# broadinstitute/colab-repeat-finder

Hardware: AMD Instinct MI355X
Metric: Gbp/s scanned (motif 1-50) (higher is better)
Workload: dtype u32 bit planes (2-bit bases)

## Files before the change

colab-repeat-finder_amd/csrc/scan_vertical.hip:

```cpp
#include <algorithm>
#include <cstdio>
#include <cstdlib>
#include <utility>
#include <vector>

#include "prf_host.h"
#include "prf_static_for.h"
#include "scan_vertical.h"
#include "verify_impl.h"

namespace {

#include "vscan_common.h"
#include "vscan_verify.h"
#include "vscan_tasks.h"

__device__ __forceinline__ void set_prio(u32 p) {
#ifdef PRF_NO_PRIO
    return;
#endif
    if (p == 0u) __builtin_amdgcn_s_setprio(0);
    else if (p == 1u) __builtin_amdgcn_s_setprio(1);
    else if (p == 2u) __builtin_amdgcn_s_setprio(2);
    else __builtin_amdgcn_s_setprio(3);
}

__device__ __forceinline__ u32 lds_add(prf_lds_u32 *p, u32 v) {
    return __hip_atomic_fetch_add(p, v, __ATOMIC_RELAXED, __HIP_MEMORY_SCOPE_WORKGROUP);
}

__device__ __forceinline__ void dma16(const void *src_lane, u32 lds_byte_off) {
    __builtin_amdgcn_global_load_lds((prf_glb_cvoid *)src_lane, (prf_lds_void *)(prf_smem + lds_byte_off), 16, 0, 0);
}

template <int NC>
struct NextRegs {
    static constexpr int extra = NC - 64;
    static constexpr u32 n_extra = (u32)(2 * RG * extra);
    static_assert(n_extra <= (u32)NTH, "one virtual-lane slot per thread");
    static_assert((RG * extra) % 64 == 0, "virtual-lane staging: one plane per wave");
    prf_u32x4 ev, en;
    u32 entry;

    __device__ __forceinline__ static prf_u32x4 ld16(const void *ubase, u32 byte_off) {
        return *reinterpret_cast<const prf_u32x4 *>(reinterpret_cast<const char *>(ubase) + byte_off);
    }
    __device__ __forceinline__ void load(const prf_vscan_args &g, u32 e, int tid, int wave, u32 r1_off) {
        e = (u32)__builtin_amdgcn_readfirstlane((int)e);
        entry = e;
        const u64 tile = e & ~PRF_LAUNCH_MIXED;
        const prf_u32x4 *ph = reinterpret_cast<const prf_u32x4 *>(g.VH) + tile * (RG * 64), *pL = reinterpret_cast<const prf_u32x4 *>(g.VL) + tile * (RG * 64);
        u32 ut = (u32)tid;
        asm volatile("" : "+v"(ut));
        {
            const u32 p = (u32)wave >> 1, rg0 = ((u32)wave & 1u) * 4u;
            const prf_u32x4 *pp = p ? pL : ph;
            const u32 l16 = (ut & 63u) * 16u;
            static_for<0, 4>([&](auto ic) {
                constexpr u32 i = (u32)decltype(ic)::value;
                dma16(reinterpret_cast<const char *>(pp) + ((rg0 + i) * 64u * 16u + l16), r1_off + ((p * RG + rg0 + i) * (u32)NC) * 16u);
            });
        }
        const prf_u32x4 z = {0, 0, 0, 0};
        ev = z;
        en = z;
        if (ut < n_extra) {
            const u32 pw = (u32)__builtin_amdgcn_readfirstlane((int)(ut / (u32)(RG * extra)));
            const u32 erg = (ut / (u32)extra) % (u32)RG, el = ut % (u32)extra;
            const u32 i0 = (erg * 64u + el) * 16u, i1 = i0 + (u32)(RG * 64) * 16u;
            if (pw == 0) {
                ev = ld16(ph, i0);
                en = ld16(ph, i1);
            } else {
                ev = ld16(pL, i0);
                en = ld16(pL, i1);
            }
        }
    }
    __device__ __forceinline__ void clear() {
        const prf_u32x4 z = {0, 0, 0, 0};
        ev = en = z;
        entry = 0;
    }
    __device__ __forceinline__ void store(prf_lds_u4 *vimg, int tid) const {
        const u32 sx = (u32)tid;
        if (sx < n_extra) {
            const u32 p = sx / (u32)(RG * extra), erg = (sx / (u32)extra) % (u32)RG, el = sx % (u32)extra;
            vimg[p * RG * NC + erg * (u32)NC + 64u + el] = (ev >> 1) | (en << 31);
        }
    }
};

__device__ __forceinline__ u32 vscan_skip(const prf_vscan_args &g) {
#ifdef PRF_DIAG
    return g.skip;
#else
    (void)g;
    return 0u;
#endif
}

template <int NC>
__global__ __launch_bounds__(NTH, 6) void prf_vscan_kernel(prf_vscan_args g) {
    constexpr u32 R1_OFF = (u32)SMEM_HDR, R1_BYTES = (u32)(2 * RG * NC * 16);
    constexpr u32 RECS_OFF = R1_OFF + R1_BYTES, KEYS_OFF = RECS_OFF + (u32)REC_CAP * 8u, SLOW_OFF = KEYS_OFF + 2u * (u32)ROW_CAP_LDS * 4u,
                  HOTW_OFF = SLOW_OFF + (u32)SLOW_CAP * 16u, BITEMS_OFF = HOTW_OFF + (u32)FLAG_CAP * 2u;
    static_assert(SLOW_CAP * 16 >= 256, "the all-N stream masks lie in the deferred candidates' list");
    static_assert(2 * LW * 8 <= (int)R1_BYTES, "the window of the linear planes must fit the image's region");
    static_assert((2 * LW / 2 + 63) / 64 <= 5 * MAX_WAVES, "window pieces per wave");
    prf_lds_u4 *vimg = (prf_lds_u4 *)(prf_smem + R1_OFF);
    prf_lds_u64 *recs = (prf_lds_u64 *)(prf_smem + RECS_OFF);
    prf_lds_u32 *keys = (prf_lds_u32 *)(prf_smem + KEYS_OFF);
    prf_lds_u32 *nostart = (prf_lds_u32 *)(prf_smem + SLOW_OFF);
    prf_lds_u32 *hotw = (prf_lds_u32 *)(prf_smem + HOTW_OFF);
    prf_lds_u32 *bitems = (prf_lds_u32 *)(prf_smem + BITEMS_OFF);

    const int tid0 = (int)threadIdx.x;
    const int wave = __builtin_amdgcn_readfirstlane(tid0 >> 6);
    auto entry_of = [&](u32 sl) -> u32 { return g.flat_base != ~0u ? g.flat_base + sl : g.launch_list[sl]; };

    set_prio(g.plan.prio & 3u);
    NextRegs<NC> sr;
    sr.load(g, entry_of(blockIdx.x), tid0, wave, R1_OFF);
    for (u32 v = (u32)tid0; v < 8u * g.plan.n_tasks; v += (u32)NTH) {
        const prf_vtask task = g.plan.tasks[v >> 3];
        const u32 kk = v & 7u;
        if (task.kind == 0 && ((task.valid >> kk) & 1u))
            bitems[(u32)task.item0 + (u32)__builtin_popcount((u32)task.valid & ((1u << kk) - 1u))] = ((u32)task.k0 + kk) | ((u32)task.stride << 16);
    }
    {
        prf_lds_u32 *cof_lds = bitems + g.plan.n_group_k;
        for (int i = tid0; i < (int)g.plan.cof_words; i += NTH) cof_lds[i] = prf_cof_table.v[i];
    }
    if (tid0 == 0) {
        TileCtx *tcw = reinterpret_cast<TileCtx *>(prf_smem);
        tcw->H = g.H; tcw->L = g.L; tcw->X = g.X;
        tcw->E = g.E;
        tcw->slab_cap = g.slab_cap;
        tcw->min_repeats = g.min_repeats;
        tcw->min_span = g.min_span;
        tcw->lin_off = R1_OFF;
        tcw->keys_off = KEYS_OFF;
        tcw->slow_off = SLOW_OFF;
        tcw->k_exact0 = g.plan.k_exact0;
        tcw->cof_off = BITEMS_OFF + 4u * g.plan.n_group_k;
    }

    const u32 xcd = blockIdx.x & 7u;
    const u32 first_ticket = (gridDim.x - xcd + 7u) >> 3;
    u64 *ticket_word = g.counters + (PRF_CNT_SHARD0 + xcd * PRF_CNT_SHARD_STRIDE + PRF_SH_TILE_TICKET);
    prf_lds_u32 *next_words = (prf_lds_u32 *)(prf_smem + HDR_NEXT);
    u32 slot_next = 0;
    u32 parity = 0;
    prf_lds_u32 *wg_stats = (prf_lds_u32 *)(prf_smem + HDR_STATS);
    if (tid0 == 0) wg_stats[0] = wg_stats[1] = 0;
    for (u32 slot = blockIdx.x; slot < g.n_launch; slot = slot_next, parity ^= 1u) {
    int wave_s = wave;
    asm volatile("" : "+s"(wave_s));
    u32 ones = ~0u;
    asm volatile("" : "+s"(ones));
    int tid = wave_s * 64 + (int)__builtin_amdgcn_mbcnt_hi(ones, __builtin_amdgcn_mbcnt_lo(ones, 0u));
    asm volatile("" : "+v"(tid));
    const int lane = tid & 63;
    const u32 entry = sr.entry;
    const bool hasx = (entry & PRF_LAUNCH_MIXED) != 0;
    const u64 tile = entry & ~PRF_LAUNCH_MIXED;
    prf_lds_u32 *cnt = smem_cnt(parity);

    PRF_STAMP(0);
#ifdef PRF_STAMPS
    if (g.dbg && lane == 0) g.dbg[((u64)slot * MAX_WAVES + wave) * 16 + 12] = __builtin_amdgcn_s_memrealtime();
#endif
    set_prio(g.plan.prio & 3u);
    {
        sr.store(vimg, tid);
        if (hasx && tid < 64) {
            const u32 *px = reinterpret_cast<const u32 *>(g.X + tile * PRF_TILE_WORDS);
            u32 m = 0;
#pragma unroll 1
            for (u32 b0 = 0; b0 < 32u; b0 += 8u) {
                u32 v[8];
                static_for<0, 8>([&](auto bc) { v[decltype(bc)::value] = *(prf_glb_cu32 *)(px + ((b0 + (u32)decltype(bc)::value) * 64u + (u32)tid)); });
                static_for<0, 8>([&](auto bc) { m |= (v[decltype(bc)::value] == ~0u ? 1u : 0u) << (b0 + (u32)decltype(bc)::value); });
            }
            nostart[tid] = m;
        }
        if (tid < 8) cnt[tid] = 0;
        if (tid == 0) {
            TileCtx *tcw = reinterpret_cast<TileCtx *>(prf_smem);
            tcw->w0 = tile * PRF_TILE_WORDS - LIN_PRE;
            tcw->xz_lo = hasx ? 0 : tile * PRF_TILE;
            tcw->xz_hi = hasx ? 0 : (tile + 2) * PRF_TILE;
            tcw->slab = (prf_glb_u64 *)(g.slabs + (u64)slot * g.slab_cap);
            tcw->tile_base = tile * PRF_TILE;
            tcw->has_lin = 0u;
            tcw->cnt_off = (u32)HDR_CNT + 32u * parity;
        }
    }
    PRF_STAMP(1);
    __syncthreads();
    PRF_STAMP(2);

    set_prio(((g.plan.slack_waves >> wave) & 1u) ? (g.plan.prio >> 4) & 3u : (g.plan.prio >> 2) & 3u);
    Emit em;
    em.recs = recs;
    em.cnt = cnt;
    em.lane = lane;
#ifdef PRF_STAMPS
    u64 *task_dbg = g.dbg ? g.dbg + ((u64)slot * MAX_WAVES + wave) * 16 : nullptr;
#else
    u64 *task_dbg = nullptr;
#endif
    {
        u32 allow = hasx ? ~nostart[lane] : ~0u;
        if (vscan_skip(g) & 1u) allow = 0u;
        run_tasks<NC>((prf_lds_cu4 *)vimg, hotw, g.plan, wave, lane, hasx, allow, em, task_dbg);
    }
    constexpr u32 WIN_UNITS = (u32)LW;
    constexpr u32 WIN_PIECES = (WIN_UNITS + 63u) / 64u;
    static_assert(WIN_PIECES == 17, "the window's pieces are dealt 9 + 8 to the first two waves to arrive");
    prf_u32x4 wv[9];
    u32 order = 0;
    {
        if (lane == 0) order = atomicAdd((u32 *)(cnt + CNT_ROWS0), 1u);
        order = (u32)__builtin_amdgcn_readfirstlane((int)order);
        const long long w0 = (long long)(tile * PRF_TILE_WORDS) - LIN_PRE;
        const u64 *wh = g.H + w0, *wl = g.L + w0;
        const prf_u32x4 z = {0, 0, 0, 0};
        static_for<0, 9>([&](auto ic) { wv[decltype(ic)::value] = z; });
        if (order < 2u) {
            const u32 first = order * 9u, n = order ? 8u : 9u;
            static_for<0, 9>([&](auto ic) {
                constexpr u32 i = (u32)decltype(ic)::value;
                if (i < n) {
                    const u32 u = (first + i) * 64u + (u32)lane;
                    const u64 *src = u < (u32)LW / 2u ? wh + 2u * u : wl + 2u * (u - (u32)LW / 2u);
                    if (u < WIN_UNITS) wv[i] = *reinterpret_cast<const prf_u32x4 *>(src);
                }
            });
        }
    }
    u64 ticket = 0;
    const bool ticket_thread = order == 0u && lane == 0;
    if (ticket_thread) ticket = atomicAdd(ticket_word, 1ull);
    PRF_STAMP(3);
    __syncthreads();
    {
        if (order < 2u) {
            const u32 first = order * 9u, n = order ? 8u : 9u;
            static_for<0, 9>([&](auto ic) {
                constexpr u32 i = (u32)decltype(ic)::value;
                if (i < n) {
                    const u32 u = (first + i) * 64u + (u32)lane;
                    if (u < WIN_UNITS) *(prf_lds_u4 *)(prf_smem + R1_OFF + 16u * u) = wv[i];
                }
            });
        }
        const u32 n0 = cnt[CNT_ROWS];
        for (u32 i = (u32)tid; i < (u32)ROW_CAP_LDS; i += (u32)NTH)
            if (i >= n0) keys[i] = 0xFFFFFFFFu;
        if (tid == 0) {
            reinterpret_cast<TileCtx *>(prf_smem)->has_lin = 1u;
            cnt[CNT_ROWS0] = n0;
            cnt[CNT_LONG0] = cnt[CNT_LONG];
        }
    }
    u32 slot_pre = 0, entry_pre = entry;
    if (ticket_thread) {
        slot_pre = (first_ticket + (u32)ticket) * 8u + xcd;
        if (slot_pre < g.n_launch) entry_pre = entry_of(slot_pre);
    }
    __syncthreads();
    PRF_STAMP(4);

    set_prio(wave < MAX_WAVES / 2 ? (g.plan.prio >> 6) & 3u : (g.plan.prio >> 8) & 3u);
    const u32 *xw = hasx ? reinterpret_cast<const u32 *>(g.X + ((long long)(tile * PRF_TILE_WORDS) - LIN_PRE)) : nullptr;
    typedef const unsigned short __attribute__((address_space(3))) prf_lds_cu16;
    u32 n_recs = cnt[CNT_RECS], n_flags = cnt[CNT_FLAGS];
    {
        if (tid == 0) {
            const u32 early = cnt[CNT_EARLY];
            wg_stats[0] += n_flags + n_recs + early;
            wg_stats[1] += early;
        }
        n_recs = n_recs < (u32)REC_CAP ? n_recs : (u32)REC_CAP;
        n_flags = n_flags < (u32)FLAG_CAP ? n_flags : (u32)FLAG_CAP;
#ifdef PRF_STAMPS
        if (g.dbg && tid == 0) g.dbg[((u64)slot * MAX_WAVES + 0) * 16 + 11] = (u64)n_flags | ((u64)n_recs << 32);
#endif
        if (vscan_skip(g) & 2u) n_flags = 0;
        if (vscan_skip(g) & 4u) n_recs = 0;
        verify_all((prf_lds_cu64 *)recs, n_recs, (prf_lds_cu32 *)bitems, (vscan_skip(g) & 8u) ? 0u : g.plan.n_group_k, (prf_lds_cu16 *)hotw, n_flags, xw, (u32)tid, task_dbg);
    }
    set_prio((g.plan.prio >> 10) & 3u);
    if (ticket_thread) {
        next_words[0] = slot_pre;
        next_words[1] = entry_pre;
    }
    PRF_STAMP(5);
    __syncthreads();
    {
        const u32 n_slow = (u32)__builtin_amdgcn_readfirstlane((int)cnt[CNT_SLOW]);
        if (n_slow) {
            if (n_slow <= (u32)SLOW_CAP) {
                if ((u32)tid < n_slow) {
                    prf_lds_u64 *slow = (prf_lds_u64 *)(prf_smem + SLOW_OFF);
                    slow_item(slow[2u * (u32)tid], slow[2u * (u32)tid + 1u]);
                }
            } else {
                if (tid == 0) {
                    cnt[CNT_ROWS] = cnt[CNT_ROWS0];
                    cnt[CNT_LONG] = cnt[CNT_LONG0];
                }
                __syncthreads();
                verify_general((prf_lds_cu64 *)recs, n_recs, (prf_lds_cu32 *)bitems, g.plan.n_group_k, (prf_lds_cu16 *)hotw, n_flags, (u32)tid);
            }
            __syncthreads();
        }
    }
    PRF_STAMP(6);
    const u64 nw = *(prf_lds_u64 *)next_words;
    slot_next = (u32)__builtin_amdgcn_readfirstlane((int)(u32)nw);
    const u32 entry_next = (u32)(nw >> 32);
    const u32 n_rows = (vscan_skip(g) & 16u) ? 0u : (u32)__builtin_amdgcn_readfirstlane((int)cnt[CNT_ROWS]);
    const u32 n_long = (u32)__builtin_amdgcn_readfirstlane((int)cnt[CNT_LONG]);
    u64 *slab = g.slabs + (u64)slot * g.slab_cap;
    const u32 n_store = n_rows < g.slab_cap ? n_rows : g.slab_cap;
    bool unsorted = false;
    if (tid == 0) {
        g.slab_count[slot] = n_rows;
        if (n_store && !(vscan_skip(g) & 32u)) atomicAdd(&g.block_sum[slot >> g.gather_shift], n_store);
    }

    if (n_rows > (u32)ROW_CAP_LDS) {
        constexpr u32 R1_ROWS = R1_BYTES / 8u;
        static_assert(R1_ROWS % 32u == 0, "padding of the dense-tile key list");
        if (n_store <= R1_ROWS) {
            prf_lds_u32 *k2 = (prf_lds_u32 *)(prf_smem + R1_OFF), *v2 = k2 + R1_ROWS;
            for (u32 i = (u32)tid; i < (u32)ROW_CAP_LDS; i += (u32)NTH) {
                k2[i] = keys[i];
                v2[i] = keys[ROW_CAP_LDS + i];
            }
            for (u32 i = (u32)ROW_CAP_LDS + (u32)tid; i < n_store; i += (u32)NTH) {
                const u64 r = slab[i];
                k2[i] = (u32)r;
                v2[i] = (u32)(r >> 32);
            }
            for (u32 i = n_store + (u32)tid; i < ((n_store + 31u) & ~31u); i += (u32)NTH) k2[i] = 0xFFFFFFFFu;
            __syncthreads();
            typedef __attribute__((address_space(3))) const prf_u32x4 prf_lds_ckey4;
            prf_lds_ckey4 *k4 = (prf_lds_ckey4 *)k2;
            for (u32 r = (u32)tid; r < n_store; r += (u32)NTH) {
                const u32 mine = k2[r], kv = v2[r];
                u32 rank = 0;
                for (u32 c0 = 0; 4u * c0 < n_store; c0 += 8u) {
#pragma unroll
                    for (u32 j = 0; j < 8u; j++) {
                        const prf_u32x4 v = k4[c0 + j];
                        rank += (v.x < mine ? 1u : 0u) + (v.y < mine ? 1u : 0u) + (v.z < mine ? 1u : 0u) + (v.w < mine ? 1u : 0u);
                    }
                }
                slab[rank] = (u64)mine | ((u64)kv << 32);
            }
            __syncthreads();
        } else {
            for (u32 i = (u32)tid; i < (u32)ROW_CAP_LDS && i < n_store; i += (u32)NTH) slab[i] = (u64)keys[i] | ((u64)keys[ROW_CAP_LDS + i] << 32);
            unsorted = true;
        }
    }

    if (slot_next < g.n_launch) sr.load(g, entry_next, tid, wave, R1_OFF);
    else sr.clear();

    if (n_rows && n_rows <= (u32)ROW_CAP_LDS) {
        const u32 lg = n_rows > 128u ? 0u : (n_rows > 64u ? 1u : (n_rows > 32u ? 2u : 3u));
        const u32 P = 1u << lg, part = (u32)tid & (P - 1u);
        typedef __attribute__((address_space(3))) const prf_u32x4 prf_lds_ckey4;
        prf_lds_ckey4 *k4 = (prf_lds_ckey4 *)keys;
        for (u32 row0 = 0; row0 < n_rows; row0 += (u32)NTH >> lg) {
            const u32 row = row0 + ((u32)tid >> lg);
            const u32 r = row < n_rows ? row : 0u;
            const u32 mine = keys[r];
            const u32 kv = keys[ROW_CAP_LDS + r];
            u32 rank = 0;
            for (u32 c0 = part; 4u * c0 < n_rows; c0 += 8u * P) {
                prf_u32x4 v[8];
#pragma unroll
                for (u32 j = 0; j < 8u; j++) v[j] = k4[c0 + j * P];
                asm volatile("" : "+v"(v[0]), "+v"(v[1]), "+v"(v[2]), "+v"(v[3]), "+v"(v[4]), "+v"(v[5]), "+v"(v[6]), "+v"(v[7]));
#pragma unroll
                for (u32 j = 0; j < 8u; j++) {
                    rank += v[j].x < mine ? 1u : 0u;
                    rank += v[j].y < mine ? 1u : 0u;
                    rank += v[j].z < mine ? 1u : 0u;
                    rank += v[j].w < mine ? 1u : 0u;
                }
            }
            if (P >= 2u) rank += (u32)__builtin_amdgcn_update_dpp(0, (int)rank, 0xB1, 0xF, 0xF, true);
            if (P >= 4u) rank += (u32)__builtin_amdgcn_update_dpp(0, (int)rank, 0x4E, 0xF, 0xF, true);
            if (P >= 8u) rank += (u32)__builtin_amdgcn_update_dpp(0, (int)rank, 0x141, 0xF, 0xF, true);
            if (row < n_rows && part == 0 && rank < g.slab_cap && !(vscan_skip(g) & 64u)) slab[rank] = (u64)mine | ((u64)kv << 32);
        }
    }
    if ((u32)tid < n_long && (u32)tid < PRF_LONG_PER_TILE)
        g.long_ends[(u64)slot * PRF_LONG_PER_TILE + (u32)tid] = ((prf_lds_u64 *)(prf_smem + HDR_LONG))[tid];
    if (tid == 0) {
        if (n_rows > g.slab_cap) atomicMax(&g.counters[PRF_CNT_HIT_OVF], (u64)n_rows);
        if (unsorted) atomicMax(&g.counters[PRF_CNT_UNSORTED], 1ull);
        if (n_long > PRF_LONG_PER_TILE) atomicMax(&g.counters[PRF_CNT_LONG_OVF], (u64)n_long);
    }
    PRF_STAMP(7);
#ifdef PRF_STAMPS
    if (g.dbg && lane == 0) g.dbg[((u64)slot * MAX_WAVES + wave) * 16 + 13] = __builtin_amdgcn_s_memrealtime();
#endif
    }
    if (tid0 == 0) {
        const u64 cand_total = wg_stats[0], early_total = wg_stats[1];
        if (cand_total) atomicAdd(&g.counters[PRF_CNT_SHARD0 + (blockIdx.x % PRF_CNT_NSHARD) * PRF_CNT_SHARD_STRIDE + PRF_SH_CAND], cand_total);
        if (early_total) atomicAdd(&g.counters[PRF_CNT_SHARD0 + (blockIdx.x % PRF_CNT_NSHARD) * PRF_CNT_SHARD_STRIDE + PRF_SH_EARLY], early_total);
    }
}

}

static u32 resident_per_cu(u32 nc, u32 lds) {
    int n = 0;
    hipError_t e = nc == 72 ? hipOccupancyMaxActiveBlocksPerMultiprocessor(&n, prf_vscan_kernel<72>, NTH, lds)
                            : hipOccupancyMaxActiveBlocksPerMultiprocessor(&n, prf_vscan_kernel<80>, NTH, lds);
    if (e != hipSuccess || n < 1) {
        (void)hipGetLastError();
        n = (int)std::max(1u, (160u * 1024u) / std::max(1u, lds + 1280u));
    }
    return (u32)std::min(n, 6);
}

hipError_t prf_vertical_launch(hipStream_t s, const prf_vscan_args &args) {
    if (args.n_launch == 0) return hipSuccess;
    u32 lds = args.plan.lds_bytes;
#ifdef PRF_DIAG
    static const u32 lds_pad = getenv("PRF_LDS_PAD") ? (u32)atoi(getenv("PRF_LDS_PAD")) : 0u;
    lds += lds_pad;
#endif
    static int n_cu = 0;
    if (n_cu == 0) {
        int dev = 0;
        hipDeviceProp_t prop;
        if (hipGetDevice(&dev) != hipSuccess || hipGetDeviceProperties(&prop, dev) != hipSuccess) return hipErrorInvalidDevice;
        n_cu = prop.multiProcessorCount;
    }
    static u32 cache_lds = ~0u, cache_nc = 0, cache_per_cu = 0;
    if (cache_lds != lds || cache_nc != args.plan.nc) {
        cache_per_cu = resident_per_cu(args.plan.nc, lds);
        cache_lds = lds;
        cache_nc = args.plan.nc;
#ifdef PRF_DIAG
        if (getenv("PRF_DEBUG")) fprintf(stderr, "[prf] fused kernel: nc %u, %u bytes of LDS, %u workgroups per CU\n", args.plan.nc, lds, cache_per_cu);
#endif
    }
    const dim3 grid(std::min(args.n_launch, cache_per_cu * (u32)n_cu)), block(NTH);
    switch (args.plan.nc) {
        case 72: hipLaunchKernelGGL((prf_vscan_kernel<72>), grid, block, lds, s, args); break;
        case 80: hipLaunchKernelGGL((prf_vscan_kernel<80>), grid, block, lds, s, args); break;
        default: return hipErrorInvalidValue;
    }
    return hipGetLastError();
}
```

colab-repeat-finder_amd/csrc/vscan_verify.h:

```cpp

__device__ __forceinline__ void emit_row(const TileCtx &tc, u64 a, u64 b, u32 k) {
    const u64 span = b + k - a;
    prf_lds_u32 *cnt = (prf_lds_u32 *)(prf_smem + tc.cnt_off);
    u32 kv = k;
    if (span >= 65535ull) {
        const u32 j = atomicAdd((u32 *)(cnt + CNT_LONG), 1u);
        if (j < PRF_LONG_PER_TILE) {
            ((prf_lds_u64 *)(prf_smem + HDR_LONG))[j] = b + k;
            kv |= (j + 1u) << 16;
        }
    }
    const u32 key = ((u32)(a - tc.tile_base) << 16) | (span < 65535ull ? (u32)span : 65535u);
    const u32 i = atomicAdd((u32 *)(cnt + CNT_ROWS), 1u);
    if (i < (u32)ROW_CAP_LDS) {
        prf_lds_u32 *keys = (prf_lds_u32 *)(prf_smem + tc.keys_off);
        keys[i] = key;
        keys[ROW_CAP_LDS + i] = kv;
    } else if (i < tc.slab_cap) {
        tc.slab[i] = (u64)key | ((u64)kv << 32);
    }
}

__device__ __noinline__ u64 tile_mismatch64(u64 q, u32 k) {
    const TileCtx &tc = *reinterpret_cast<const TileCtx *>(prf_smem);
    prf_window_view view;
    view.lds = (prf_lds_cu64 *)(prf_smem + tc.lin_off);
    view.w0 = tc.w0;
    view.nwords = tc.has_lin ? LW : 0;
    view.xz_lo = tc.xz_lo;
    view.xz_hi = tc.xz_hi;
    view.x_in_lds = 0;
    view.P[0] = tc.H; view.P[1] = tc.L; view.P[2] = tc.X;
    view.E = tc.E;
    return view.mismatch64(q, k);
}

__device__ __forceinline__ u64 run_end(u64 from, u32 k) {
    u64 b = from;
    for (;;) {
        const u64 m2 = tile_mismatch64(b, k);
        if (m2) return b + (u64)__builtin_ctzll(m2);
        b += 64;
    }
}

__device__ __forceinline__ bool motif_is_repeat(u64 a, u32 k) {
    const TileCtx &tc = *reinterpret_cast<const TileCtx *>(prf_smem);
    for (u32 cf = ((prf_lds_cu32 *)(prf_smem + tc.cof_off))[k]; cf; cf >>= 8) {
        const u32 d = cf & 255u, need = k - d;
        bool has = true;
        for (u32 off = 0; off < need; off += 64) {
            u64 mm = tile_mismatch64(a + off, d);
            const u32 left = need - off;
            if (left < 64) mm &= (1ull << left) - 1ull;
            if (mm) {
                has = false;
                break;
            }
        }
        if (has) return true;
    }
    return false;
}

__device__ __noinline__ void verify_stream(u64 sp, u32 k, u32 sc) {
    const TileCtx &tc = *reinterpret_cast<const TileCtx *>(prf_smem);
    const long long M = prf_min_matches(k, tc.min_repeats, tc.min_span);
    if (sc == 0) {
        const u64 m = sp ? tile_mismatch64(sp - 1, k) : ((tile_mismatch64(0, k) << 1) | 1ull);
        u64 r = ~m;
        u32 len = 1;
        while (2 * len <= (u32)M) {
            r &= r >> len;
            len *= 2;
        }
        if (len < (u32)M) r &= r >> ((u32)M - len);
        u64 st = r & (m << 1) & 0x1FFFFFFFEull;
        while (st) {
            const u32 i = (u32)__builtin_ctzll(st);
            st &= st - 1;
            const u64 a = sp - 1 + i;
            const u64 after = m >> i;
            const u64 b = after ? a + (u64)__builtin_ctzll(after) : run_end(a + (64 - i), k);
            if (!motif_is_repeat(a, k)) emit_row(tc, a, b, k);
        }
        return;
    }
    const u32 S = 1u << (sc - 1u);
    const u32 back = 8u * S;
    for (u32 j = 0; j < 4u; j += S) {
        const u64 p = sp + 8u * j;
        const u32 look = p >= back ? back : (u32)p;
        const u64 mm = tile_mismatch64(p - look, k);
        if ((mm >> look) & 0xFFull) continue;
        const u64 lead = mm & ((1ull << look) - 1ull);
        u64 a;
        if (lead == 0) {
            if (look == back) continue;
            a = p - look;
        } else {
            a = p - (u64)__builtin_clzll(lead << (64 - look));
        }
        if (a < tc.tile_base) continue;
        const u64 seen = (mm >> look) >> 8;
        const u64 b = seen ? p + 8 + (u64)__builtin_ctzll(seen) : run_end(p + (64 - look), k);
        if ((long long)(b - a) < M) continue;
        if (!motif_is_repeat(a, k)) emit_row(tc, a, b, k);
    }
}

constexpr u32 WIN_POS = (u32)LW * 64u;

__device__ __forceinline__ u32 look32(prf_lds_cu32 *plane, u32 q) {
    const u32 w = q >> 5;
    return __builtin_amdgcn_alignbit(plane[w + 1], plane[w], q & 31u);
}
__device__ __forceinline__ u64 look64(prf_lds_cu32 *plane, u32 q) {
    const u32 w = q >> 5, sft = q & 31u;
    const u32 w0 = plane[w], w1 = plane[w + 1], w2 = plane[w + 2];
    return (u64)__builtin_amdgcn_alignbit(w1, w0, sft) | ((u64)__builtin_amdgcn_alignbit(w2, w1, sft) << 32);
}
__device__ __forceinline__ u32 xword(const u32 *xw, u32 w) {
    return *(prf_glb_cu32 *)(reinterpret_cast<const char *>(xw) + 4u * w);
}
__device__ __forceinline__ u32 xlook32(const u32 *xw, u32 q) {
    const u32 w = q >> 5;
    return __builtin_amdgcn_alignbit(xword(xw, w + 1), xword(xw, w), q & 31u);
}
__device__ __forceinline__ u64 xlook64(const u32 *xw, u32 q) {
    const u32 w = q >> 5, sft = q & 31u;
    const u32 w0 = xword(xw, w), w1 = xword(xw, w + 1), w2 = xword(xw, w + 2);
    return (u64)__builtin_amdgcn_alignbit(w1, w0, sft) | ((u64)__builtin_amdgcn_alignbit(w2, w1, sft) << 32);
}
struct WinCtx {
    prf_lds_cu32 *h, *l, *cof;
    const u32 *xw;
    u64 win0;
    u32 min_repeats, min_span;
};

__device__ __forceinline__ u32 win_mismatch32(const WinCtx &wc, u32 q, u32 k) {
    u32 r = (look32(wc.h, q) ^ look32(wc.h, q + k)) | (look32(wc.l, q) ^ look32(wc.l, q + k));
    if (wc.xw) r |= xlook32(wc.xw, q) | xlook32(wc.xw, q + k);
    return r;
}
__device__ __forceinline__ u64 win_mismatch64(const WinCtx &wc, u32 q, u32 k) {
    u64 r = (look64(wc.h, q) ^ look64(wc.h, q + k)) | (look64(wc.l, q) ^ look64(wc.l, q + k));
    if (wc.xw) r |= xlook64(wc.xw, q) | xlook64(wc.xw, q + k);
    return r;
}

__device__ __forceinline__ u32 min_matches32(u32 k, u32 min_repeats, u32 min_span) {
    const u32 a = (min_repeats - 1u) * k, b = min_span > k ? min_span - k : 0u;
    return a > b ? a : b;
}

__device__ __forceinline__ void defer(const TileCtx &tc, u64 a, u32 k, u32 sc, u32 whole_stream, u32 need_motif, u64 from) {
    const u32 i = atomicAdd((u32 *)((prf_lds_u32 *)(prf_smem + tc.cnt_off) + CNT_SLOW), 1u);
    if (i < (u32)SLOW_CAP) {
        prf_lds_u64 *slow = (prf_lds_u64 *)(prf_smem + tc.slow_off);
        slow[2u * i] = a | ((u64)k << 40) | ((u64)sc << 49) | ((u64)whole_stream << 51) | ((u64)need_motif << 52);
        slow[2u * i + 1u] = from;
    }
}

__device__ __noinline__ void slow_item(u64 w0, u64 from) {
    const TileCtx &tc = *reinterpret_cast<const TileCtx *>(prf_smem);
    const u64 a = w0 & ((1ull << 40) - 1ull);
    const u32 k = (u32)(w0 >> 40) & 511u, sc = (u32)(w0 >> 49) & 3u;
    if ((w0 >> 51) & 1ull) {
        verify_stream(a, k, sc);
        return;
    }
    if (((w0 >> 52) & 1ull) && motif_is_repeat(a, k)) return;
    const u64 b = run_end(from, k);
    if ((long long)(b - a) < prf_min_matches(k, tc.min_repeats, tc.min_span)) return;
    emit_row(tc, a, b, k);
}

__device__ __forceinline__ bool win_run_end(const WinCtx &wc, u32 &from, u32 k, u64 &b) {
    for (;;) {
        if (from + k + 96u > WIN_POS) return false;
        const u64 m2 = win_mismatch64(wc, from, k);
        if (m2) {
            b = wc.win0 + from + (u64)__builtin_ctzll(m2);
            return true;
        }
        from += 64u;
    }
}

__device__ __forceinline__ bool win_motif_is_repeat(const WinCtx &wc, u32 a, u32 k) {
    for (u32 cf = wc.cof[k]; cf; cf >>= 8) {
        const u32 d = cf & 255u, need = k - d;
        bool has = true;
        for (u32 off = 0; off < need; off += 32) {
            u32 mm = win_mismatch32(wc, a + off, d);
            const u32 left = need - off;
            if (left < 32) mm &= (1u << left) - 1u;
            if (mm) {
                has = false;
                break;
            }
        }
        if (has) return true;
    }
    return false;
}

__device__ __forceinline__ u64 shr128(u64 lo, u64 hi, u32 sft) { return (lo >> sft) | (hi << (64u - sft)); }

__device__ __forceinline__ u32 small_cof(u32 k) {
    const u64 t = k < 8u ? 0x0123010201010000ull : 0x0027014601250304ull;
    return (u32)(t >> (8u * (k & 7u))) & 255u;
}

__device__ __forceinline__ void win_verify_flag(const TileCtx &tc, const WinCtx &wc, u32 rl, u32 bit, u32 k) {
    const u32 q = WIN_LEAD + (bit * 64u + rl) * T;
    const u32 w = (q - 1u) >> 5, sft = (q - 1u) & 31u;
    const u32 a0 = wc.h[w], a1 = wc.h[w + 1], a2 = wc.h[w + 2], a3 = wc.h[w + 3], a4 = wc.h[w + 4];
    const u32 b0 = wc.l[w], b1 = wc.l[w + 1], b2 = wc.l[w + 2], b3 = wc.l[w + 3], b4 = wc.l[w + 4];
    const u64 hlo = (u64)__builtin_amdgcn_alignbit(a1, a0, sft) | ((u64)__builtin_amdgcn_alignbit(a2, a1, sft) << 32);
    const u64 hhi = (u64)__builtin_amdgcn_alignbit(a3, a2, sft) | ((u64)__builtin_amdgcn_alignbit(a4, a3, sft) << 32);
    const u64 llo = (u64)__builtin_amdgcn_alignbit(b1, b0, sft) | ((u64)__builtin_amdgcn_alignbit(b2, b1, sft) << 32);
    const u64 lhi = (u64)__builtin_amdgcn_alignbit(b3, b2, sft) | ((u64)__builtin_amdgcn_alignbit(b4, b3, sft) << 32);
    u64 xlo = 0, xhi = 0;
    if (wc.xw) {
        const u32 c0 = xword(wc.xw, w), c1 = xword(wc.xw, w + 1), c2 = xword(wc.xw, w + 2), c3 = xword(wc.xw, w + 3), c4 = xword(wc.xw, w + 4);
        xlo = (u64)__builtin_amdgcn_alignbit(c1, c0, sft) | ((u64)__builtin_amdgcn_alignbit(c2, c1, sft) << 32);
        xhi = (u64)__builtin_amdgcn_alignbit(c3, c2, sft) | ((u64)__builtin_amdgcn_alignbit(c4, c3, sft) << 32);
    }
    const u32 M = min_matches32(k, wc.min_repeats, wc.min_span);
    const u64 m = (hlo ^ shr128(hlo, hhi, k)) | (llo ^ shr128(llo, lhi, k)) | xlo | shr128(xlo, xhi, k);
    u64 r = ~m;
    if (M >= 2) r &= r >> 1;
    if (M >= 4) r &= r >> 2;
    if (M >= 8) r &= r >> 4;
    {
        const u32 len = M >= 8 ? 8u : (M >= 4 ? 4u : (M >= 2 ? 2u : 1u));
        r &= r >> (M - len);
    }
    u64 st = r & (m << 1) & 0x1FFFFFFFEull;
    const u32 cof_k = small_cof(k);
    while (st) {
        const u32 i = (u32)__builtin_ctzll(st);
        st &= st - 1;
        bool rep = false;
        for (u32 cf = cof_k; cf && !rep; cf >>= 4) {
            const u32 d = cf & 15u;
            const u64 md = (hlo ^ shr128(hlo, hhi, d)) | (llo ^ shr128(llo, lhi, d));
            rep = ((md >> i) & ((1ull << (k - d)) - 1ull)) == 0;
        }
        if (rep) continue;
        const u32 a = q - 1u + i;
        const u64 after = m >> i;
        if (after) {
            emit_row(tc, wc.win0 + a, wc.win0 + a + (u64)__builtin_ctzll(after), k);
        } else {
            u32 from = a + (64u - i);
            u64 b;
            if (win_run_end(wc, from, k, b)) emit_row(tc, wc.win0 + a, b, k);
            else defer(tc, wc.win0 + a, k, 0u, 0u, 0u, wc.win0 + from);
        }
    }
}

__device__ __forceinline__ void win_verify_group(const TileCtx &tc, const WinCtx &wc, u32 q, u32 k, u32 S) {
    const u32 M = min_matches32(k, wc.min_repeats, wc.min_span);
    const u32 back = 8u * S;
    const u64 m = win_mismatch64(wc, q - 32u, k);
    const u32 cof_k = wc.cof[k];
    u32 leaders = 0;
    u32 nbs = 0;
    for (u32 j = 0; j < 4u; j += S) {
        const u32 gb = 32u + 8u * j;
        const u64 lead = m << (64u - gb);
        const u32 nb = lead ? (u32)__builtin_clzll(lead) : 64u;
        const bool ok = ((m >> gb) & 0xFFull) == 0 && nb < back && q - 32u + gb - nb >= WIN_LEAD;
        leaders |= (ok ? 1u : 0u) << j;
        nbs |= (nb & 31u) << (5u * j);
    }
    while (leaders) {
        const u32 j = (u32)__builtin_ctz(leaders);
        leaders &= leaders - 1;
        const u32 gb = 32u + 8u * j, nb = (nbs >> (5u * j)) & 31u;
        const u32 a = q - 32u + gb - nb;
        if (a + 2u * k + 96u > WIN_POS) {
            defer(tc, wc.win0 + a, k, 0u, 0u, 1u, wc.win0 + (q - 32u + gb + 8u));
            continue;
        } else {
            const u32 d1 = cof_k & 255u, d2 = (cof_k >> 8) & 255u, d3 = (cof_k >> 16) & 255u;
            const u32 mm1 = win_mismatch32(wc, a, d1 ? d1 : 1u);
            const u32 mm2 = win_mismatch32(wc, a, d2 ? d2 : 1u);
            const u32 mm3 = win_mismatch32(wc, a, d3 ? d3 : 1u);
            bool rep = false;
            for (u32 ci = 0; ci < 4u && !rep; ci++) {
                const u32 d = (cof_k >> (8u * ci)) & 255u;
                if (d == 0) break;
                const u32 need = k - d;
                u32 mm = ci == 0 ? mm1 : (ci == 1 ? mm2 : (ci == 2 ? mm3 : win_mismatch32(wc, a, d)));
                if (need < 32) mm &= (1u << need) - 1u;
                rep = mm == 0;
                for (u32 off = 32; off < need && rep; off += 32) {
                    u32 m2 = win_mismatch32(wc, a + off, d);
                    const u32 left = need - off;
                    if (left < 32) m2 &= (1u << left) - 1u;
                    rep = m2 == 0;
                }
            }
            if (rep) continue;
        }
        const u64 seen = gb + 8u < 64u ? m >> (gb + 8u) : 0ull;
        u64 b;
        if (seen) {
            b = wc.win0 + (q - 32u + gb + 8u) + (u64)__builtin_ctzll(seen);
        } else {
            const u64 m2 = win_mismatch64(wc, q + 32u, k);
            if (m2) {
                b = wc.win0 + (q + 32u) + (u64)__builtin_ctzll(m2);
            } else {
                u32 from = q + 96u;
                if (!win_run_end(wc, from, k, b)) {
                    defer(tc, wc.win0 + a, k, 0u, 0u, 0u, wc.win0 + from);
                    continue;
                }
            }
        }
        if (b - (wc.win0 + a) < (u64)M) continue;
        emit_row(tc, wc.win0 + a, b, k);
    }
}

__device__ __forceinline__ void boundary_item(const TileCtx &tc, const WinCtx &wc, u32 k, u32 S) {
    const u64 tile_end = tc.tile_base + PRF_TILE;
    const u32 back = 8u * S;
    const u64 mm = win_mismatch64(wc, WIN_LEAD + PRF_TILE - 32u, k);
    const u32 lo = (u32)mm;
    const u32 c = lo ? (u32)__builtin_clz(lo) : 32u;
    if (c == 0 || c >= back) return;
    const u64 a = tile_end - c;
    const u64 hi = mm >> 32;
    u64 b;
    if (hi) {
        b = tile_end + (u64)__builtin_ctzll(hi);
    } else {
        u32 from = WIN_LEAD + PRF_TILE + 32u;
        if (!win_run_end(wc, from, k, b)) {
            defer(tc, a, k, 0u, 0u, 1u, wc.win0 + from);
            return;
        }
    }
    if (b - a < (u64)min_matches32(k, tc.min_repeats, tc.min_span)) return;
    static_assert(WIN_LEAD + PRF_TILE + 2u * PRF_VMAX_K + 96u <= WIN_POS, "the motif of a boundary item lies inside the window");
    if (!win_motif_is_repeat(wc, WIN_LEAD + PRF_TILE - c, k)) emit_row(tc, a, b, k);
}

__device__ __forceinline__ void boundary_general(const TileCtx &tc, u32 k, u32 S) {
    const u64 tile_end = tc.tile_base + PRF_TILE;
    const u32 back = 8u * S;
    const u64 mm = tile_mismatch64(tile_end - 32, k);
    const u32 lo = (u32)mm;
    const u32 c = lo ? (u32)__builtin_clz(lo) : 32u;
    if (c == 0 || c >= back) return;
    const u64 a = tile_end - c;
    const u64 hi = mm >> 32;
    const u64 b = hi ? tile_end + (u64)__builtin_ctzll(hi) : run_end(tile_end + 32, k);
    if (b - a < (u64)min_matches32(k, tc.min_repeats, tc.min_span)) return;
    if (!motif_is_repeat(a, k)) emit_row(tc, a, b, k);
}

__device__ __forceinline__ prf_lds_u32 *smem_cnt(u32 parity) { return (prf_lds_u32 *)(prf_smem + HDR_CNT) + 8u * parity; }

__device__ __forceinline__ void verify_all(prf_lds_cu64 *recs, u32 n_recs, prf_lds_cu32 *bitems, u32 n_bitems, const unsigned short __attribute__((address_space(3))) *flags,
                                           u32 n_flags, const u32 *xw, u32 tid, u64 *dbg) {
#ifdef PRF_STAMPS
#define PRF_VSTAMP(i) do { if (dbg && (tid & 63u) == 0) dbg[i] = __builtin_amdgcn_s_memtime(); } while (0)
#else
#define PRF_VSTAMP(i) do { } while (0)
#endif
    const TileCtx &tc = *reinterpret_cast<const TileCtx *>(prf_smem);
    WinCtx wc;
    wc.h = (prf_lds_cu32 *)(prf_smem + tc.lin_off);
    wc.l = wc.h + 2 * LW;
    wc.xw = xw;
    wc.cof = (prf_lds_cu32 *)(prf_smem + tc.cof_off);
    wc.win0 = tc.tile_base - WIN_LEAD;
    wc.min_repeats = tc.min_repeats;
    wc.min_span = tc.min_span;
    if (tid >= (u32)NTH / 2u) {
        const u32 up = (u32)NTH - 1u - tid;
        for (u32 idx = 2u * (up & 63u) + (up >> 6); idx < n_recs; idx += (u32)NTH / 2u) {
            const u64 rec = recs[idx];
            const u32 rl = (u32)rec & 63u, k = ((u32)rec >> 6) & 511u, sc = ((u32)rec >> 15) & 3u;
            u32 word = (u32)(rec >> 17);
            while (word) {
                const u32 bit = (u32)__builtin_ctz(word);
                word &= word - 1;
                const u32 sq = (bit * 64u + rl) * T;
                if (sq >= 32u || xw) win_verify_group(tc, wc, WIN_LEAD + sq, k, 1u << (sc - 1u));
                else defer(tc, tc.tile_base, k, sc, 1u, 0u, 0ull);
            }
        }
    } else {
        for (u32 idx = tid; idx < n_flags; idx += (u32)NTH / 2u) {
            const u32 f = flags[idx], frl = f & 63u, fbit = (f >> 6) & 31u, k = tc.k_exact0 + (f >> 11);
            if ((frl | fbit) || xw) win_verify_flag(tc, wc, frl, fbit, k);
            else defer(tc, tc.tile_base, k, 0u, 1u, 0u, 0ull);
        }
        PRF_VSTAMP(14);
        for (u32 idx = (u32)NTH / 2u - 1u - tid; idx < n_bitems; idx += (u32)NTH / 2u) {
            const u32 it = bitems[idx];
            boundary_item(tc, wc, it & 0xFFFFu, it >> 16);
        }
    }
}

__device__ __noinline__ void verify_general(prf_lds_cu64 *recs, u32 n_recs, prf_lds_cu32 *bitems, u32 n_bitems,
                                            const unsigned short __attribute__((address_space(3))) *flags, u32 n_flags, u32 tid) {
    const TileCtx &tc = *reinterpret_cast<const TileCtx *>(prf_smem);
    for (u32 idx = tid; idx < n_flags; idx += (u32)NTH) {
        const u32 f = flags[idx], frl = f & 63u, fbit = (f >> 6) & 31u, k = tc.k_exact0 + (f >> 11);
        verify_stream(tc.tile_base + (u64)(fbit * 64u + frl) * T, k, 0u);
    }
    for (u32 idx = tid; idx < n_recs; idx += (u32)NTH) {
        const u64 rec = recs[idx];
        const u32 rl = (u32)rec & 63u, k = ((u32)rec >> 6) & 511u, sc = ((u32)rec >> 15) & 3u;
        u32 word = (u32)(rec >> 17);
        while (word) {
            const u32 bit = (u32)__builtin_ctz(word);
            word &= word - 1;
            verify_stream(tc.tile_base + (u64)(bit * 64u + rl) * T, k, sc);
        }
    }
    for (u32 idx = tid; idx < n_bitems; idx += (u32)NTH) {
        const u32 it = bitems[idx];
        boundary_general(tc, it & 0xFFFFu, it >> 16);
    }
}
```

Measured before the change: 5735.

## Compact record-wave verification work into per-wave LDS lists for lane balancing

Record-verifying waves now expand each record's candidate bits into a per-wave LDS list, using ballot and mbcnt prefix sums. The list is then processed 64 items at a time so every lane gets one stream. This removes the divergence from lanes looping over different popcounts. Leader verification now uses 64-bit mismatch windows with LDS loads batched ahead of use, and far-window candidates are deferred up front. The cost is extra LDS traffic, wave barriers, and list-capacity logic in the region behind the window, plus register pressure from the packed leader items.

```diff
diff --git a/colab-repeat-finder_amd/csrc/scan_vertical.hip b/colab-repeat-finder_amd/csrc/scan_vertical.hip
--- a/colab-repeat-finder_amd/csrc/scan_vertical.hip
+++ b/colab-repeat-finder_amd/csrc/scan_vertical.hip
@@ -108,6 +108,7 @@
     static_assert(SLOW_CAP * 16 >= 256, "the all-N stream masks lie in the deferred candidates' list");
     static_assert(2 * LW * 8 <= (int)R1_BYTES, "the window of the linear planes must fit the image's region");
     static_assert((2 * LW / 2 + 63) / 64 <= 5 * MAX_WAVES, "window pieces per wave");
+    static_assert(LEAD_OFF == R1_OFF + 2u * (u32)LW * 8u && LEAD_OFF + 2u * LEAD_CAP * 4u <= R1_OFF + R1_BYTES, "the record waves' stream lists lie in R1 behind the window");
     prf_lds_u4 *vimg = (prf_lds_u4 *)(prf_smem + R1_OFF);
     prf_lds_u64 *recs = (prf_lds_u64 *)(prf_smem + RECS_OFF);
     prf_lds_u32 *keys = (prf_lds_u32 *)(prf_smem + KEYS_OFF);
diff --git a/colab-repeat-finder_amd/csrc/vscan_verify.h b/colab-repeat-finder_amd/csrc/vscan_verify.h
--- a/colab-repeat-finder_amd/csrc/vscan_verify.h
+++ b/colab-repeat-finder_amd/csrc/vscan_verify.h
@@ -132,6 +132,16 @@
     const u32 w0 = xword(xw, w), w1 = xword(xw, w + 1), w2 = xword(xw, w + 2);
     return (u64)__builtin_amdgcn_alignbit(w1, w0, sft) | ((u64)__builtin_amdgcn_alignbit(w2, w1, sft) << 32);
 }
+typedef u32 prf_u32x3 __attribute__((ext_vector_type(3)));
+__device__ __forceinline__ prf_u32x3 raw64(prf_lds_cu32 *plane, u32 q) {
+    const u32 w = q >> 5;
+    const prf_u32x3 r = {plane[w], plane[w + 1], plane[w + 2]};
+    return r;
+}
+__device__ __forceinline__ u64 cut64(prf_u32x3 r, u32 q) {
+    const u32 sft = q & 31u;
+    return (u64)__builtin_amdgcn_alignbit(r.y, r.x, sft) | ((u64)__builtin_amdgcn_alignbit(r.z, r.y, sft) << 32);
+}
 struct WinCtx {
     prf_lds_cu32 *h, *l, *cof;
     const u32 *xw;
@@ -265,70 +275,88 @@
     }
 }
 
-__device__ __forceinline__ void win_verify_group(const TileCtx &tc, const WinCtx &wc, u32 q, u32 k, u32 S) {
-    const u32 M = min_matches32(k, wc.min_repeats, wc.min_span);
+constexpr u32 LEAD_CAP = 192u;
+constexpr u32 LEAD_OFF = (u32)SMEM_HDR + 2u * (u32)LW * 8u;
+constexpr u32 LEAD_NO_END = 31u;
+
+__device__ __forceinline__ u32 win_leaders(const WinCtx &wc, u32 q, u32 k, u32 S, u64 m, u32 &nbs, u32 &far) {
     const u32 back = 8u * S;
-    const u64 m = win_mismatch64(wc, q - 32u, k);
-    const u32 cof_k = wc.cof[k];
     u32 leaders = 0;
-    u32 nbs = 0;
-    for (u32 j = 0; j < 4u; j += S) {
+    nbs = 0;
+    far = 0;
+#pragma unroll
+    for (u32 j = 0; j < 4u; j++) {
         const u32 gb = 32u + 8u * j;
         const u64 lead = m << (64u - gb);
         const u32 nb = lead ? (u32)__builtin_clzll(lead) : 64u;
-        const bool ok = ((m >> gb) & 0xFFull) == 0 && nb < back && q - 32u + gb - nb >= WIN_LEAD;
-        leaders |= (ok ? 1u : 0u) << j;
+        const u32 a = q - 32u + gb - nb;
+        const bool ok = (j & (S - 1u)) == 0u && ((m >> gb) & 0xFFull) == 0 && nb < back && a >= WIN_LEAD;
+        const bool out = a + 2u * k + 96u > WIN_POS;
+        leaders |= (ok && !out ? 1u : 0u) << j;
+        far |= (ok && out ? 1u : 0u) << j;
         nbs |= (nb & 31u) << (5u * j);
     }
-    while (leaders) {
-        const u32 j = (u32)__builtin_ctz(leaders);
-        leaders &= leaders - 1;
-        const u32 gb = 32u + 8u * j, nb = (nbs >> (5u * j)) & 31u;
-        const u32 a = q - 32u + gb - nb;
-        if (a + 2u * k + 96u > WIN_POS) {
-            defer(tc, wc.win0 + a, k, 0u, 0u, 1u, wc.win0 + (q - 32u + gb + 8u));
-            continue;
-        } else {
-            const u32 d1 = cof_k & 255u, d2 = (cof_k >> 8) & 255u, d3 = (cof_k >> 16) & 255u;
-            const u32 mm1 = win_mismatch32(wc, a, d1 ? d1 : 1u);
-            const u32 mm2 = win_mismatch32(wc, a, d2 ? d2 : 1u);
-            const u32 mm3 = win_mismatch32(wc, a, d3 ? d3 : 1u);
-            bool rep = false;
-            for (u32 ci = 0; ci < 4u && !rep; ci++) {
-                const u32 d = (cof_k >> (8u * ci)) & 255u;
-                if (d == 0) break;
-                const u32 need = k - d;
-                u32 mm = ci == 0 ? mm1 : (ci == 1 ? mm2 : (ci == 2 ? mm3 : win_mismatch32(wc, a, d)));
-                if (need < 32) mm &= (1u << need) - 1u;
-                rep = mm == 0;
-                for (u32 off = 32; off < need && rep; off += 32) {
-                    u32 m2 = win_mismatch32(wc, a + off, d);
-                    const u32 left = need - off;
-                    if (left < 32) m2 &= (1u << left) - 1u;
-                    rep = m2 == 0;
-                }
-            }
-            if (rep) continue;
-        }
-        const u64 seen = gb + 8u < 64u ? m >> (gb + 8u) : 0ull;
-        u64 b;
-        if (seen) {
-            b = wc.win0 + (q - 32u + gb + 8u) + (u64)__builtin_ctzll(seen);
-        } else {
-            const u64 m2 = win_mismatch64(wc, q + 32u, k);
-            if (m2) {
-                b = wc.win0 + (q + 32u) + (u64)__builtin_ctzll(m2);
-            } else {
-                u32 from = q + 96u;
-                if (!win_run_end(wc, from, k, b)) {
-                    defer(tc, wc.win0 + a, k, 0u, 0u, 0u, wc.win0 + from);
-                    continue;
-                }
-            }
-        }
-        if (b - (wc.win0 + a) < (u64)M) continue;
-        emit_row(tc, wc.win0 + a, b, k);
-    }
+    return leaders;
+}
+
+__device__ __forceinline__ u64 make_leader(u32 q, u32 k, u32 cof_k, u32 j, u32 nb, u64 m) {
+    const u32 gb = 32u + 8u * j;
+    const u64 seen = gb + 8u < 64u ? m >> (gb + 8u) : 0ull;
+    const u32 e = seen ? (u32)__builtin_ctzll(seen) : LEAD_NO_END;
+    const u32 lo = (q - 32u + gb - nb) | (k << 17) | (nb << 26) | ((cof_k >> 24) ? 1u << 31 : 0u);
+    const u32 hi = (cof_k & 0xFFFFFFu) | (j << 24) | (e << 26);
+    return (u64)lo | ((u64)hi << 32);
+}
+
+__device__ __forceinline__ bool win_has_period(const WinCtx &wc, u32 a, u32 k, u32 d, u64 mm) {
+    const u32 need = k - d;
+    if (need < 64u) mm &= (1ull << need) - 1ull;
+    bool has = mm == 0;
+    for (u32 off = 64; off < need && has; off += 64) {
+        u64 m2 = win_mismatch64(wc, a + off, d);
+        const u32 left = need - off;
+        if (left < 64u) m2 &= (1ull << left) - 1ull;
+        has = m2 == 0;
+    }
+    return has;
+}
+
+__device__ __forceinline__ void win_verify_leader(const TileCtx &tc, const WinCtx &wc, u64 item) {
+    const u32 lo = (u32)item, hi = (u32)(item >> 32);
+    const u32 a = lo & 0x1FFFFu, k = (lo >> 17) & 511u, nb = (lo >> 26) & 31u;
+    const u32 d1 = hi & 255u, d2 = (hi >> 8) & 255u, d3 = (hi >> 16) & 255u, j = (hi >> 24) & 3u, e = (hi >> 26) & 31u;
+    const u32 ge = a + nb + 8u;
+    const u32 q32 = ge + 24u - 8u * j;
+    const u32 p1 = a + (d1 ? d1 : 1u), p2 = a + (d2 ? d2 : 1u);
+    prf_u32x3 ra = raw64(wc.h, a), sa = raw64(wc.l, a), r1 = raw64(wc.h, p1), s1 = raw64(wc.l, p1), r2 = raw64(wc.h, p2), s2 = raw64(wc.l, p2);
+    asm volatile("" : "+v"(ra), "+v"(sa), "+v"(r1), "+v"(s1), "+v"(r2), "+v"(s2));
+    const u64 ha = cut64(ra, a), la = cut64(sa, a);
+    u64 mm1 = (ha ^ cut64(r1, p1)) | (la ^ cut64(s1, p1)), mm2 = (ha ^ cut64(r2, p2)) | (la ^ cut64(s2, p2));
+    if (wc.xw) {
+        const u64 xa = xlook64(wc.xw, a);
+        mm1 |= xa | xlook64(wc.xw, p1);
+        mm2 |= xa | xlook64(wc.xw, p2);
+    }
+    bool rep = d1 && win_has_period(wc, a, k, d1, mm1);
+    if (!rep && d2) rep = win_has_period(wc, a, k, d2, mm2);
+    if (!rep && d3) rep = win_has_period(wc, a, k, d3, win_mismatch64(wc, a, d3));
+    if (!rep && (lo >> 31)) {
+        const u32 d4 = wc.cof[k] >> 24;
+        rep = win_has_period(wc, a, k, d4, win_mismatch64(wc, a, d4));
+    }
+    if (rep) return;
+    u64 b;
+    if (e != LEAD_NO_END) {
+        b = wc.win0 + ge + e;
+    } else {
+        u32 from = q32;
+        if (!win_run_end(wc, from, k, b)) {
+            defer(tc, wc.win0 + a, k, 0u, 0u, 0u, wc.win0 + from);
+            return;
+        }
+    }
+    if (b - (wc.win0 + a) < (u64)min_matches32(k, wc.min_repeats, wc.min_span)) return;
+    emit_row(tc, wc.win0 + a, b, k);
 }
 
 __device__ __forceinline__ void boundary_item(const TileCtx &tc, const WinCtx &wc, u32 k, u32 S) {
@@ -389,17 +417,74 @@
     wc.min_span = tc.min_span;
     if (tid >= (u32)NTH / 2u) {
         const u32 up = (u32)NTH - 1u - tid;
-        for (u32 idx = 2u * (up & 63u) + (up >> 6); idx < n_recs; idx += (u32)NTH / 2u) {
-            const u64 rec = recs[idx];
-            const u32 rl = (u32)rec & 63u, k = ((u32)rec >> 6) & 511u, sc = ((u32)rec >> 15) & 3u;
-            u32 word = (u32)(rec >> 17);
-            while (word) {
-                const u32 bit = (u32)__builtin_ctz(word);
-                word &= word - 1;
-                const u32 sq = (bit * 64u + rl) * T;
-                if (sq >= 32u || xw) win_verify_group(tc, wc, WIN_LEAD + sq, k, 1u << (sc - 1u));
-                else defer(tc, tc.tile_base, k, sc, 1u, 0u, 0ull);
+        const u32 hwl = tid & 63u;
+        prf_lds_u32 *list = (prf_lds_u32 *)(prf_smem + LEAD_OFF) + (up >> 6) * LEAD_CAP;
+        u32 idx = 2u * (up & 63u) + (up >> 6), word = 0, head = 0;
+        for (;;) {
+            u32 n_items = 0;
+            bool more;
+            for (;;) {
+                if (word == 0u && idx < n_recs) {
+                    const u64 rec = recs[idx];
+                    idx += (u32)NTH / 2u;
+                    head = (u32)rec & 0x1FFFFu;
+                    word = (u32)(rec >> 17);
+                }
+                const u32 pc = (u32)__builtin_popcount(word);
+                u32 at = n_items, total = 0;
+#pragma unroll
+                for (u32 b = 0; b < 6u; b++) {
+                    const u64 bal = __builtin_amdgcn_ballot_w64(((pc >> b) & 1u) != 0);
+                    at += __builtin_amdgcn_mbcnt_hi((u32)(bal >> 32), __builtin_amdgcn_mbcnt_lo((u32)bal, 0)) << b;
+                    total += (u32)__builtin_popcountll(bal) << b;
+                }
+                u32 room = at < LEAD_CAP ? LEAD_CAP - at : 0u;
+                for (; word && room; room--) {
+                    const u32 bit = (u32)__builtin_ctz(word);
+                    word &= word - 1;
+                    list[at++] = (bit * 64u + (head & 63u)) | ((head >> 6) << 11);
+                }
+                n_items = n_items + total < LEAD_CAP ? n_items + total : LEAD_CAP;
+                more = __builtin_amdgcn_ballot_w64(word != 0u || idx < n_recs) != 0ull;
+                if (!more || n_items == LEAD_CAP) break;
             }
+            __builtin_amdgcn_fence(__ATOMIC_RELEASE, "wavefront");
+            __builtin_amdgcn_wave_barrier();
+            PRF_VSTAMP(14);
+            for (u32 i0 = 0; i0 < n_items; i0 += 64u) {
+                u32 leaders = 0, nbs = 0, far = 0, cof_k = 0, q = 0, k = 0;
+                u64 m = 0;
+                if (i0 + hwl < n_items) {
+                    const u32 it = list[i0 + hwl], sq = (it & 2047u) * T, sc = (it >> 20) & 3u;
+                    k = (it >> 11) & 511u;
+                    q = WIN_LEAD + sq;
+                    if (sq >= 32u || xw) {
+                        prf_u32x3 r0 = raw64(wc.h, q - 32u), r1 = raw64(wc.l, q - 32u), r2 = raw64(wc.h, q - 32u + k), r3 = raw64(wc.l, q - 32u + k);
+                        cof_k = wc.cof[k];
+                        asm volatile("" : "+v"(r0), "+v"(r1), "+v"(r2), "+v"(r3), "+v"(cof_k));
+                        m = (cut64(r0, q - 32u) ^ cut64(r2, q - 32u + k)) | (cut64(r1, q - 32u) ^ cut64(r3, q - 32u + k));
+                        if (xw) m |= xlook64(xw, q - 32u) | xlook64(xw, q - 32u + k);
+                        leaders = win_leaders(wc, q, k, 1u << (sc - 1u), m, nbs, far);
+                        while (far) {
+                            const u32 j = (u32)__builtin_ctz(far);
+                            far &= far - 1;
+                            defer(tc, wc.win0 + (q + 8u * j - ((nbs >> (5u * j)) & 31u)), k, 0u, 0u, 1u, wc.win0 + (q + 8u * j + 8u));
+                        }
+                    } else {
+                        defer(tc, tc.tile_base, k, sc, 1u, 0u, 0ull);
+                    }
+                }
+                while (__builtin_amdgcn_ballot_w64(leaders != 0u) != 0ull) {
+                    if (leaders) {
+                        const u32 j = (u32)__builtin_ctz(leaders);
+                        leaders &= leaders - 1;
+                        win_verify_leader(tc, wc, make_leader(q, k, cof_k, j, (nbs >> (5u * j)) & 31u, m));
+                    }
+                }
+            }
+            if (!more) break;
+            __builtin_amdgcn_fence(__ATOMIC_RELEASE, "wavefront");
+            __builtin_amdgcn_wave_barrier();
         }
     } else {
         for (u32 idx = tid; idx < n_flags; idx += (u32)NTH / 2u) {
```

Result: faster. 5854, median of 6 (+2.1%).
